# shizukutanaka/Otedama

Measured on AMD Instinct MI355X. Metric: hashes/sec (whole node) SHA-256d + scrypt at 1/2/4/8 MI355X; p50 share latency, higher is better.
Workload: dtype u32

## Files before the change

### csrc/bindings.cpp

```cpp
#include <pybind11/pybind11.h>
#include <pybind11/stl.h>

#include <array>
#include <atomic>
#include <cstring>
#include <stdexcept>
#include <thread>
#include <tuple>

#include "otedama/aead.h"
#include "otedama/job.h"
#include "otedama/runtime.h"
#include "otedama/trace.h"
#include "otedama/sha256.h"
#include "otedama/sv2_frame.h"
#include "otedama/clock_bounds.h"
#include "otedama/launch_plan.h"
#include "otedama/search_launch.h"
#include "otedama/work_queue.h"
#include "otedama/x11.h"

namespace py = pybind11;
using namespace otedama;

// ... 286 lines not shown
                       &status);
        }
        py::list frames(k);
        for (size_t i = 0; i < k; ++i) {
          const Sv2FrameRec& r = recs[i];
          frames[i] = py::make_tuple(r.extension_type, r.msg_type, r.offset, r.length);
        }
        return py::make_tuple(frames, consumed, status);
      },
      py::arg("buf"), py::arg("max_frame"),
      "Split complete SV2 frames: ([(extension_type, msg_type, payload_offset, payload_length)], consumed, status)");
  m.def("cpu_scan_sha256d", [](const py::bytes& h, const py::bytes& t, uint32_t start, uint64_t count) {
    std::string hs = need(h, 80, "header"), ts = need(t, 32, "target");
    std::vector<uint32_t> hits;
    {
      py::gil_scoped_release r;
      hits = cpu_scan_sha256d(reinterpret_cast<const uint8_t*>(hs.data()), reinterpret_cast<const uint8_t*>(ts.data()),
                              start, count);
    }
    return hits;
  }, py::arg("header"), py::arg("target"), py::arg("start"), py::arg("count"));
  m.def("cpu_scan_method", &cpu_scan_method);
  m.def("_cpu_scan_lanes", [](int lanes, const py::bytes& h, const py::bytes& t, uint32_t start, uint64_t count) {
    std::string hs = need(h, 80, "header"), ts = need(t, 32, "target");
    std::vector<uint32_t> hits;
    {
      py::gil_scoped_release r;
      hits = cpu_scan_sha256d_lanes(lanes, reinterpret_cast<const uint8_t*>(hs.data()),
                                    reinterpret_cast<const uint8_t*>(ts.data()), start, count);
    }
    return hits;
  });
  m.def("merkle_root", [](const py::dict& job, uint64_t en2) {
    auto j = make_job(job); uint8_t root[32];
    merkle_root_from_coinbase(*j, en2, root);
    return to_bytes(root, 32);
  });
  m.def("variant_header", [](const py::dict& job, uint64_t v) {
    auto j = make_job(job);
    uint8_t hdr[80]; uint32_t ver, nt; uint64_t en2;
    j->variant_header(v, hdr, &ver, &nt, &en2);
    return py::make_tuple(to_bytes(hdr, 80), ver, nt, en2);
  });
  m.def("variant_space", [](const py::dict& job) { return make_job(job)->variant_space(); });

  m.def("sha256d_prepare", [](const py::bytes& h, const py::bytes& t) {
    std::string hs = need(h, 80, "header"), ts = need(t, 32, "target");
    Sha256dParams p;
    sha256d_prepare(reinterpret_cast<const uint8_t*>(hs.data()), reinterpret_cast<const uint8_t*>(ts.data()), &p);
    return py::bytes(reinterpret_cast<const char*>(&p), sizeof p);
  });
  m.attr("SHA256D_MAX_K") = kSha256dMaxK;
  {
    py::list ks;
    for (int k = 2; k <= kSha256dMaxK; ++k)
      if (sha256d_k_floor(k) == k) ks.append(k);
    m.attr("SHA256D_K_VALUES") = py::tuple(ks);
  }
  m.def("sha256d_prepare_k", [](const py::list& headers, const py::bytes& t) {
    std::string ts = need(t, 32, "target");
    std::vector<std::string> hs;
    for (auto& h : headers) hs.push_back(need(h.cast<py::bytes>(), 80, "header"));
    std::vector<const uint8_t*> ptrs;
    for (auto& h : hs) ptrs.push_back(reinterpret_cast<const uint8_t*>(h.data()));
    Sha256dParamsK p;
    if (!sha256d_prepare_k(ptrs.data(), (int)ptrs.size(), reinterpret_cast<const uint8_t*>(ts.data()), &p))
      throw std::invalid_argument("need K headers (K in SHA256D_K_VALUES) with identical bytes 64..75");
    return py::bytes(reinterpret_cast<const char*>(&p), sizeof p);
  }, py::arg("headers"), py::arg("target"));
  m.attr("SHA256D_V_GROUP") = kSha256dVGroup;
  m.attr("SHA256D_V2_GROUP") = kSha256dV2Group;
  m.def("sha256d_prepare_v", [](const py::list& headers, const py::bytes& t) {
    std::string ts = need(t, 32, "target");
    std::vector<std::string> hs;
    for (auto& h : headers) hs.push_back(need(h.cast<py::bytes>(), 80, "header"));
    std::vector<const uint8_t*> ptrs;
    for (auto& h : hs) ptrs.push_back(reinterpret_cast<const uint8_t*>(h.data()));
    Sha256dParamsV p;
    std::vector<Sha256dVariant> vars(hs.size());
    if (!sha256d_prepare_v(ptrs.data(), (int)ptrs.size(), reinterpret_cast<const uint8_t*>(ts.data()), &p, vars.data()))
      throw std::invalid_argument("need a positive multiple of 64 headers with identical bytes 64..75");
    return py::make_tuple(py::bytes(reinterpret_cast<const char*>(&p), sizeof p),
                          py::bytes(reinterpret_cast<const char*>(vars.data()), vars.size() * sizeof(Sha256dVariant)));
  }, py::arg("headers"), py::arg("target"));
  m.def("scrypt_prepare", [](const py::bytes& h, const py::bytes& t) {
    std::string hs = need(h, 80, "header"), ts = need(t, 32, "target");
    ScryptParams p;
    scrypt_prepare(reinterpret_cast<const uint8_t*>(hs.data()), reinterpret_cast<const uint8_t*>(ts.data()), &p);
    return py::bytes(reinterpret_cast<const char*>(&p), sizeof p);
  });

  m.def("x11_prepare", [](const py::bytes& h, const py::bytes& t) {
    std::string hs = need(h, 80, "header"), ts = need(t, 32, "target");
    X11Params p;
    x11_prepare(reinterpret_cast<const uint8_t*>(hs.data()), reinterpret_cast<const uint8_t*>(ts.data()), &p);
    return py::bytes(reinterpret_cast<const char*>(&p), sizeof p);
  });

  m.def("trace_push", [](const std::string& name) { trace_push(name.c_str()); });
  m.def("trace_pop", [] { trace_pop(); });
  m.def("trace_mark", [](const std::string& name) { trace_mark(name.c_str()); });
  m.def("gpu_device_count", &gpu_device_count);
  m.def("gpu_arch_name", &gpu_arch_name);
  m.def("gpu_cu_count", &gpu_cu_count);
  m.def("scrypt_scratch_bytes", &scrypt_scratch_bytes);
  m.def("maps_range_writable", [](const std::string& maps, uint64_t lo, uint64_t hi) {
    return maps_range_writable(maps, uintptr_t(lo), uintptr_t(hi));
  });
  m.def("launch_sha256d", [](const py::bytes& params, uint32_t base, uint64_t count, uintptr_t out, uint32_t cap,
                             int grid, uintptr_t stream) {
    std::string ps = need(params, sizeof(Sha256dParams), "params");
    Sha256dParams p; std::memcpy(&p, ps.data(), sizeof p);
    if (count == 0 || count > (1ull << 32)) throw std::invalid_argument("count must be in [1, 2^32]");
    if (grid <= 0 || out == 0) throw std::invalid_argument("bad grid / out");
    py_launch_sha256d(p, base, count, out, cap, grid, stream);
  }, py::arg("params"), py::arg("base"), py::arg("count"), py::arg("out"), py::arg("cap"), py::arg("grid"),
     py::arg("stream"));
  m.def("launch_sha256d_k", [](const py::bytes& params, uint32_t base, uint64_t count, uintptr_t out, uint32_t cap,
                               int grid, uintptr_t stream) {
    std::string ps = need(params, sizeof(Sha256dParamsK), "params");
    Sha256dParamsK p; std::memcpy(&p, ps.data(), sizeof p);
    if (p.k < 2 || p.k > kSha256dMaxK) throw std::invalid_argument("bad K");
    if (count == 0 || count > (1ull << 32)) throw std::invalid_argument("count must be in [1, 2^32]");
    if (grid <= 0 || out == 0) throw std::invalid_argument("bad grid / out");
    py_launch_sha256d_k(p, base, count, out, cap, grid, stream);
  }, py::arg("params"), py::arg("base"), py::arg("count"), py::arg("out"), py::arg("cap"), py::arg("grid"),
     py::arg("stream"));
  m.def("launch_sha256d_v", [](const py::bytes& params, uintptr_t vars, uint32_t base, uint64_t count, uintptr_t out,
                               uint32_t cap, int grid, uintptr_t stream, bool occupancy8, int block, int chains) {
    std::string ps = need(params, sizeof(Sha256dParamsV), "params");
    Sha256dParamsV p; std::memcpy(&p, ps.data(), sizeof p);
    p.occupancy8 = occupancy8 ? 1u : 0u;
    if (p.groups == 0 || count == 0 || count > (1ull << 32)) throw std::invalid_argument("bad groups / count");
    if (block != 64 && block != 256) throw std::invalid_argument("block must be 64 or 256 threads");
    if (chains < 1 || chains > 4) throw std::invalid_argument("chains must be 1..4");
    if (p.groups % uint32_t(chains) != 0)
      throw std::invalid_argument("chains variants per lane need a multiple of 64 * chains variants");
    if (grid <= 0 || (uint64_t(grid) * uint32_t(block / 64)) % (p.groups / uint32_t(chains)) != 0 || vars == 0 || out == 0)
      throw std::invalid_argument("the wave count must be a multiple of the variant groups; vars/out must be set");
    py_launch_sha256d_v(p, vars, base, count, out, cap, grid, stream, block, chains);
  }, py::arg("params"), py::arg("vars"), py::arg("base"), py::arg("count"), py::arg("out"), py::arg("cap"),
     py::arg("grid"), py::arg("stream"), py::arg("occupancy8") = false, py::arg("block") = 256, py::arg("chains") = 1);
  m.def("launch_scrypt", [](const py::bytes& params, uint32_t base, uint32_t count, uintptr_t xbuf, uintptr_t scratch,
                            int gap, uintptr_t out, uint32_t cap, int grid, uintptr_t stream) {
    std::string ps = need(params, sizeof(ScryptParams), "params");
    ScryptParams p; std::memcpy(&p, ps.data(), sizeof p);
    if (gap != 1 && gap != 2 && gap != 4 && gap != kScryptCoop && gap != kScryptLaneW8 && gap != kScryptCoop2 &&
        gap != kScryptCoopSplit)
      throw std::invalid_argument("gap must be 1, 2, 4, SCRYPT_COOP or SCRYPT_LANE_W8");
    if (grid <= 0 || out == 0 || xbuf == 0 || scratch == 0 || count == 0) throw std::invalid_argument("bad launch args");
    py_launch_scrypt(p, base, count, xbuf, scratch, gap, out, cap, grid, stream);
  }, py::arg("params"), py::arg("base"), py::arg("count"), py::arg("xbuf"), py::arg("scratch"), py::arg("gap"),
     py::arg("out"), py::arg("cap"), py::arg("grid"), py::arg("stream"));

  m.def("launch_x11_stage", [](const py::bytes& params, int stage, uint32_t base, uintptr_t H, uint32_t stride,
                               uint32_t n, uintptr_t out, uint32_t cap, uintptr_t stream) {
    std::string ps = need(params, sizeof(X11Params), "params");
    X11Params p; std::memcpy(&p, ps.data(), sizeof p);
    if (stage < 0 || stage >= kX11StageCount) throw std::invalid_argument("stage must be in [0, 11)");
    if (H == 0 || n == 0 || stride < n) throw std::invalid_argument("need H != 0, n > 0, stride >= n");
    py_launch_x11_stage(p, stage, base, H, stride, n, out, cap, stream);
  }, py::arg("params"), py::arg("stage"), py::arg("base"), py::arg("H"), py::arg("stride"), py::arg("n"),
     py::arg("out") = 0, py::arg("cap") = 0, py::arg("stream") = 0);
  m.def("launch_x11", [](const py::bytes& params, uint32_t base, uintptr_t H, uint32_t stride, uint32_t n,
                         uintptr_t out, uint32_t cap, uintptr_t stream) {
    std::string ps = need(params, sizeof(X11Params), "params");
    X11Params p; std::memcpy(&p, ps.data(), sizeof p);
    if (H == 0 || n == 0 || stride < n) throw std::invalid_argument("need H != 0, n > 0, stride >= n");
    py_launch_x11(p, base, H, stride, n, out, cap, stream);
  }, py::arg("params"), py::arg("base"), py::arg("H"), py::arg("stride"), py::arg("n"), py::arg("out") = 0,
     py::arg("cap") = 0, py::arg("stream") = 0);

  py::class_<MinerBase, std::shared_ptr<MinerBase>>(m, "Miner")
      .def("start", &MinerBase::start, py::call_guard<py::gil_scoped_release>())
      .def("stop", &MinerBase::stop, py::call_guard<py::gil_scoped_release>())
      .def("set_job", [](MinerBase& self, py::object job) {
        if (job.is_none()) { py::gil_scoped_release r; self.set_job(nullptr); return; }
        auto j = make_job(job.cast<py::dict>());
        py::gil_scoped_release r;
        self.set_job(j);
      })
      .def("poll", [](MinerBase& self, size_t max) {
        std::vector<ShareRecord> v;
        { py::gil_scoped_release r; v = self.poll(max); }
        return shares_to_list(std::move(v));
      }, py::arg("max") = 256)
      .def("stats", [](MinerBase& self) { return stats_to_dict(self.stats()); })
      .def("share_fd", &MinerBase::share_fd,
           "eventfd that becomes readable when shares are queued (read 8 bytes to reset, then poll())")
      .def_property_readonly("device_id", &MinerBase::device_id);

  py::class_<GpuMiner, MinerBase, std::shared_ptr<GpuMiner>>(m, "GpuMiner")
      .def(py::init<int, std::string, uint64_t, int, size_t, int>(), py::arg("device"), py::arg("device_id"),
           py::arg("batch_nonces") = (1ull << 32), py::arg("grid") = 2048, py::arg("queue_cap") = 1024,
           py::arg("sha_variants") = 128);
  py::class_<CpuMiner, MinerBase, std::shared_ptr<CpuMiner>>(m, "CpuMiner")
      .def(py::init<int, std::string, size_t>(), py::arg("threads"), py::arg("device_id") = "cpu-0",
           py::arg("queue_cap") = 1024);

  m.attr("SHA256D_PARAMS_SIZE") = sizeof(Sha256dParams);
  m.attr("SHA256D_V_PARAMS_SIZE") = sizeof(Sha256dParamsV);
  m.attr("SCRYPT_PARAMS_SIZE") = sizeof(ScryptParams);
}
```

### csrc/include/otedama/search_launch.h

```cpp
#pragma once
#include <cstdint>
#include <string>

#include "otedama/hitsink.h"
#include "otedama/job.h"

namespace otedama {

uint64_t scrypt_scratch_bytes(int grid, int gap);

int gpu_device_count();
std::string gpu_arch_name(int device);
int gpu_cu_count(int device);

void py_launch_sha256d(const Sha256dParams& p, uint32_t base, uint64_t count, uintptr_t out, uint32_t cap, int grid,
                       uintptr_t stream);
void py_launch_sha256d_k(const Sha256dParamsK& p, uint32_t base, uint64_t count, uintptr_t out, uint32_t cap, int grid,
                         uintptr_t stream);
void py_launch_sha256d_v(const Sha256dParamsV& p, uintptr_t vars, uint32_t base, uint64_t count, uintptr_t out,
                         uint32_t cap, int grid, uintptr_t stream, int block, int chains);
void py_launch_scrypt(const ScryptParams& p, uint32_t base, uint32_t count, uintptr_t xbuf, uintptr_t scratch, int gap,
                      uintptr_t out, uint32_t cap, int grid, uintptr_t stream);
void py_launch_x11_stage(const X11Params& p, int stage, uint32_t base, uintptr_t H, uint32_t stride, uint32_t n,
                         uintptr_t out, uint32_t cap, uintptr_t stream);
void py_launch_x11(const X11Params& p, uint32_t base, uintptr_t H, uint32_t stride, uint32_t n, uintptr_t out,
                   uint32_t cap, uintptr_t stream);

}

#ifdef __HIPCC__
#include <hip/hip_runtime.h>

namespace otedama {

hipError_t launch_sha256d_search(const Sha256dParams& p, uint32_t base, uint64_t count, const HitSink& sink, int grid,
                                 hipStream_t stream);
hipError_t launch_sha256d_search_k(const Sha256dParamsK& p, uint32_t base, uint64_t count, const HitSink& sink,
                                   int grid, hipStream_t stream);
hipError_t launch_sha256d_search_v(const Sha256dParamsV& p, const Sha256dVariant* vars, uint32_t base, uint64_t count,
                                   const HitSink& sink, int grid, hipStream_t stream, int block = 256, int chains = 1);

hipError_t launch_scrypt_search(const ScryptParams& p, uint32_t base, uint32_t count, void* xbuf, void* scratch,
                                int gap, const HitSink& sink, int grid, hipStream_t stream);

}
#endif
```

### csrc/kernels/scrypt_search.hip

```cpp
#include <hip/hip_runtime.h>

#include <cstdint>

#include "cdna_bitops.h"
#include "hitsink_dev.h"
#include <cstdlib>
#include <cstring>

#include "otedama/job.h"
#include "otedama/search_launch.h"

namespace {

using namespace otedama_dev;

__device__ __forceinline__ uint32_t bswap(uint32_t x) { return __builtin_bswap32(x); }

__device__ __forceinline__ void salsa20_8(uint32_t B[16]) {
  uint32_t x0 = B[0], x1 = B[1], x2 = B[2], x3 = B[3], x4 = B[4], x5 = B[5], x6 = B[6], x7 = B[7];
  uint32_t x8 = B[8], x9 = B[9], x10 = B[10], x11 = B[11], x12 = B[12], x13 = B[13], x14 = B[14], x15 = B[15];
#pragma unroll
  for (int i = 0; i < 8; i += 2) {
    x4 ^= rol(x0 + x12, 7);   x8 ^= rol(x4 + x0, 9);    x12 ^= rol(x8 + x4, 13);   x0 ^= rol(x12 + x8, 18);
    x9 ^= rol(x5 + x1, 7);    x13 ^= rol(x9 + x5, 9);   x1 ^= rol(x13 + x9, 13);   x5 ^= rol(x1 + x13, 18);
    x14 ^= rol(x10 + x6, 7);  x2 ^= rol(x14 + x10, 9);  x6 ^= rol(x2 + x14, 13);   x10 ^= rol(x6 + x2, 18);
    x3 ^= rol(x15 + x11, 7);  x7 ^= rol(x3 + x15, 9);   x11 ^= rol(x7 + x3, 13);   x15 ^= rol(x11 + x7, 18);
    x1 ^= rol(x0 + x3, 7);    x2 ^= rol(x1 + x0, 9);    x3 ^= rol(x2 + x1, 13);    x0 ^= rol(x3 + x2, 18);
    x6 ^= rol(x5 + x4, 7);    x7 ^= rol(x6 + x5, 9);    x4 ^= rol(x7 + x6, 13);    x5 ^= rol(x4 + x7, 18);
    x11 ^= rol(x10 + x9, 7);  x8 ^= rol(x11 + x10, 9);  x9 ^= rol(x8 + x11, 13);   x10 ^= rol(x9 + x8, 18);
    x12 ^= rol(x15 + x14, 7); x13 ^= rol(x12 + x15, 9); x14 ^= rol(x13 + x12, 13); x15 ^= rol(x14 + x13, 18);
  }
  B[0] += x0; B[1] += x1; B[2] += x2; B[3] += x3; B[4] += x4; B[5] += x5; B[6] += x6; B[7] += x7;
  B[8] += x8; B[9] += x9; B[10] += x10; B[11] += x11; B[12] += x12; B[13] += x13; B[14] += x14; B[15] += x15;
}

__device__ __forceinline__ void blockmix(uint32_t X[32]) {
#pragma unroll
  for (int k = 0; k < 16; ++k) X[k] ^= X[16 + k];
  salsa20_8(X);
#pragma unroll
  for (int k = 0; k < 16; ++k) X[16 + k] ^= X[k];
  salsa20_8(X + 16);
}

__device__ __forceinline__ void store_entry(uint4* __restrict__ dst, const uint32_t X[32]) {
#pragma unroll
  for (int q = 0; q < 8; ++q) dst[q] = make_uint4(X[4 * q], X[4 * q + 1], X[4 * q + 2], X[4 * q + 3]);
}
__device__ __forceinline__ void load_entry(const uint4* __restrict__ src, uint32_t T[32]) {
#pragma unroll
  for (int q = 0; q < 8; ++q) {
    const uint4 v = src[q];
    T[4 * q] = v.x; T[4 * q + 1] = v.y; T[4 * q + 2] = v.z; T[4 * q + 3] = v.w;
  }
}

__device__ __forceinline__ void hmac_states(const uint32_t key[8], uint32_t istate[8], uint32_t ostate[8]) {
  uint32_t blk[16];
#pragma unroll
  for (int i = 0; i < 8; ++i) blk[i] = key[i] ^ 0x36363636u;
#pragma unroll
  for (int i = 8; i < 16; ++i) blk[i] = 0x36363636u;
#pragma unroll
  for (int i = 0; i < 8; ++i) istate[i] = kSha256IVd[i];
  sha256_compress(istate, blk);
#pragma unroll
  for (int i = 0; i < 8; ++i) blk[i] = key[i] ^ 0x5c5c5c5cu;
#pragma unroll
  for (int i = 8; i < 16; ++i) blk[i] = 0x5c5c5c5cu;
#pragma unroll
  for (int i = 0; i < 8; ++i) ostate[i] = kSha256IVd[i];
  sha256_compress(ostate, blk);
}

__device__ __forceinline__ void hmac_outer(const uint32_t ostate[8], const uint32_t digest[8], uint32_t out[8]) {
  uint32_t blk[16];
#pragma unroll
  for (int i = 0; i < 8; ++i) blk[i] = digest[i];
  blk[8] = 0x80000000u;
#pragma unroll
  for (int i = 9; i < 15; ++i) blk[i] = 0u;
  blk[15] = 768u;
#pragma unroll
  for (int i = 0; i < 8; ++i) out[i] = ostate[i];
  sha256_compress(out, blk);
}

__device__ __forceinline__ void scrypt_pbkdf_in(const otedama::ScryptParams& p, uint32_t nonce, uint32_t X[32]) {
  uint32_t hdrbe[20];
#pragma unroll
  for (int i = 0; i < 19; ++i) hdrbe[i] = bswap(p.hdr[i]);
  hdrbe[19] = bswap(nonce);
  uint32_t key[8];
#pragma unroll
  for (int i = 0; i < 8; ++i) key[i] = p.hmid[i];
  {
    uint32_t blk[16] = {hdrbe[16], hdrbe[17], hdrbe[18], hdrbe[19], 0x80000000u, 0, 0, 0, 0, 0, 0, 0, 0, 0, 0, 640u};
    sha256_compress(key, blk);
  }
  uint32_t istate[8], ostate[8];
  hmac_states(key, istate, ostate);
  uint32_t ist2[8];
#pragma unroll
  for (int i = 0; i < 8; ++i) ist2[i] = istate[i];
  sha256_compress(ist2, hdrbe);
#pragma unroll
  for (int blkno = 1; blkno <= 4; ++blkno) {
    uint32_t st[8];
#pragma unroll
    for (int i = 0; i < 8; ++i) st[i] = ist2[i];
    uint32_t blk[16] = {hdrbe[16], hdrbe[17], hdrbe[18], hdrbe[19], uint32_t(blkno), 0x80000000u,
                        0, 0, 0, 0, 0, 0, 0, 0, 0, (64u + 84u) * 8u};
    sha256_compress(st, blk);
    uint32_t t[8];
    hmac_outer(ostate, st, t);
#pragma unroll
    for (int i = 0; i < 8; ++i) X[8 * (blkno - 1) + i] = bswap(t[i]);
  }
}

__device__ __forceinline__ uint32_t scrypt_pbkdf_out(const otedama::ScryptParams& p, uint32_t nonce,
                                                     const uint32_t X[32]) {
  uint32_t key[8];
#pragma unroll
  for (int i = 0; i < 8; ++i) key[i] = p.hmid[i];
  {
    uint32_t blk[16] = {bswap(p.hdr[16]), bswap(p.hdr[17]), bswap(p.hdr[18]), bswap(nonce), 0x80000000u,
                        0, 0, 0, 0, 0, 0, 0, 0, 0, 0, 640u};
    sha256_compress(key, blk);
  }
  uint32_t istate[8], ostate[8];
  hmac_states(key, istate, ostate);
  uint32_t st[8];
#pragma unroll
  for (int i = 0; i < 8; ++i) st[i] = istate[i];
  uint32_t blk[16];
#pragma unroll
  for (int i = 0; i < 16; ++i) blk[i] = bswap(X[i]);
  sha256_compress(st, blk);
#pragma unroll
  for (int i = 0; i < 16; ++i) blk[i] = bswap(X[16 + i]);
  sha256_compress(st, blk);
  uint32_t tail[16] = {1u, 0x80000000u, 0, 0, 0, 0, 0, 0, 0, 0, 0, 0, 0, 0, 0, (64u + 132u) * 8u};
  sha256_compress(st, tail);
  uint32_t out[8];
  hmac_outer(ostate, st, out);
  return out[7];
}

template <int GAP>
__device__ __forceinline__ void scrypt_romix(uint32_t X[32], uint4* __restrict__ Vw, uint32_t lane) {
  for (int i = 0; i < 1024; ++i) {
    if (i % GAP == 0) store_entry(Vw + ((uint64_t(i / GAP) * 64u + lane) << 3), X);
    blockmix(X);
  }
  for (int i = 0; i < 1024; ++i) {
    const uint32_t j = X[16] & 1023u;
    uint32_t T[32];
    load_entry(Vw + ((uint64_t(j / GAP) * 64u + lane) << 3), T);
    if constexpr (GAP > 1) {
// ... 237 lines not shown
        __builtin_amdgcn_make_buffer_rsrc(V + hw * (1024ull * 64u * 8u), (short)0, 1024 * 64 * 128, 0x00020000);
    uint32_t X[32];
    load_entry(xbuf + (h << 3), X);
    const uint32_t w1 = it1 < 1024u ? it1 : 1024u;
    for (uint32_t i = it0; i < w1; ++i) {
      coop_store_entry(X, rh, tile, lane, i);
      blockmix(X);
    }
    for (uint32_t i = it0 > 1024u ? it0 : 1024u; i < it1; ++i) {
      coop_v4u R[4];
      coop_issue<LCPOL>(X, rh, tile, lane, R);
      coop_consume(X, tile, lane, R);
      blockmix(X);
    }
    store_entry(xbuf + (h << 3), X);
  }
}

template <int LCPOL>
__global__ __launch_bounds__(256) __attribute__((amdgpu_waves_per_eu(4, 4))) void otd_scrypt_romix_coop2(
    uint32_t count, uint4* __restrict__ xbuf, uint4* __restrict__ V) {
  __shared__ uint4 tiles[4 * 256];
  const uint32_t lane = threadIdx.x & 63u;
  const uint64_t wave0 = (uint64_t(blockIdx.x) * blockDim.x + threadIdx.x) >> 6;
  const uint64_t nwaves = (uint64_t(gridDim.x) * blockDim.x) >> 6;
  const uint64_t wslot = (uint64_t(__builtin_amdgcn_readfirstlane(uint32_t(wave0 >> 32))) << 32) |
                         uint64_t(__builtin_amdgcn_readfirstlane(uint32_t(wave0)));
  uint4* VA = V + wslot * (2ull * 1024 * 64 * 8);
  uint4* VB = VA + 1024ull * 64 * 8;
  const __amdgpu_buffer_rsrc_t rsA = __builtin_amdgcn_make_buffer_rsrc(VA, (short)0, 1024 * 64 * 128, 0x00020000);
  const __amdgpu_buffer_rsrc_t rsB = __builtin_amdgcn_make_buffer_rsrc(VB, (short)0, 1024 * 64 * 128, 0x00020000);
  uint4* tile = tiles + __builtin_amdgcn_readfirstlane(threadIdx.x >> 6) * 256;
  for (uint64_t w = wslot; w * 128 < count; w += nwaves) {
    const uint64_t ia = w * 128 + lane, ib = ia + 64;
    uint32_t XA[32], XB[32];
    load_entry(xbuf + (ia << 3), XA);
    load_entry(xbuf + (ib << 3), XB);
    scrypt_romix_coop2<LCPOL>(XA, XB, rsA, rsB, tile, lane);
    store_entry(xbuf + (ia << 3), XA);
    store_entry(xbuf + (ib << 3), XB);
  }
}

__global__ __launch_bounds__(256) __attribute__((amdgpu_waves_per_eu(8, 8))) void otd_scrypt_romix_w8(
    uint32_t count, uint4* __restrict__ xbuf, uint4* __restrict__ V) {
  const uint64_t slot = uint64_t(blockIdx.x) * blockDim.x + threadIdx.x;
  const uint64_t nslots = uint64_t(gridDim.x) * blockDim.x;
  uint4* Vw = V + (slot >> 6) * (1024ull * 64u * 8u);
  const uint32_t lane = uint32_t(slot & 63u);
  for (uint64_t i = slot; i < count; i += nslots) {
    uint32_t X[32];
    load_entry(xbuf + (i << 3), X);
    scrypt_romix<1>(X, Vw, lane);
    store_entry(xbuf + (i << 3), X);
  }
}

extern "C" __global__ __launch_bounds__(256) void otd_scrypt_pbkdf_out(const otedama::ScryptParams p, uint32_t base,
                                                                       uint32_t count, const uint4* __restrict__ xbuf,
                                                                       const otedama::HitSink sink) {
  const uint32_t i = blockIdx.x * blockDim.x + threadIdx.x;
  if (i >= count) return;
  if (abort_newer(abort_peek(sink), sink.epoch)) return;
  uint32_t X[32];
  load_entry(xbuf + (uint64_t(i) << 3), X);
  const uint32_t h7 = scrypt_pbkdf_out(p, base + i, X);
  if (bswap(h7) <= p.target_hi) hit_publish(sink, base + i, 0u);
}

template __global__ void otd_scrypt_romix<1>(uint32_t, uint4*, uint4*);
template __global__ void otd_scrypt_romix<2>(uint32_t, uint4*, uint4*);
template __global__ void otd_scrypt_romix<4>(uint32_t, uint4*, uint4*);

namespace otedama {

uint64_t scrypt_scratch_bytes(int grid, int gap) {
  if (gap == kScryptCoop2) return uint64_t(grid) * 512ull * 1024ull * 128ull;
  if (gap == kScryptCoop || gap == kScryptLaneW8 || gap == kScryptCoopSplit) gap = 1;
  return uint64_t(grid) * 256ull * (1024ull / uint64_t(gap)) * 128ull;
}

static bool scrypt_write_polls() {
  static const bool on = [] {
    const char* v = std::getenv("OTEDAMA_SCRYPT_POLL");
    return !(v && v[0] == '0');
  }();
  return on;
}

static uint32_t scrypt_segments() {
  const char* v = std::getenv("OTEDAMA_SCRYPT_SEGMENTS");
  if (!v || !v[0]) return 0;
  const long x = std::strtol(v, nullptr, 10);
  return uint32_t(x < 1 ? 1 : (x > 64 ? 64 : x));
}

static int scrypt_seg_grid(int grid) {
  const char* v = std::getenv("OTEDAMA_SCRYPT_SEG_GRID");
  if (!v || !v[0]) return grid;
  int cap = 0;
  if (std::strcmp(v, "resident") == 0) {
    int dev = 0, cus = 0;
    if (hipGetDevice(&dev) != hipSuccess ||
        hipDeviceGetAttribute(&cus, hipDeviceAttributeMultiprocessorCount, dev) != hipSuccess || cus <= 0)
      return grid;
    cap = cus * 8;
  } else {
    cap = int(std::strtol(v, nullptr, 10));
  }
  return cap > 0 && cap < grid ? cap : grid;
}

hipError_t launch_scrypt_search(const ScryptParams& p, uint32_t base, uint32_t count, void* xbuf, void* scratch,
                                int gap, const HitSink& sink, int grid, hipStream_t stream) {
  uint4* X = static_cast<uint4*>(xbuf);
  uint4* V = static_cast<uint4*>(scratch);
  const int eg = int((count + 255) / 256);
  const uint32_t count64 = (count + 63u) & ~63u;
  if (gap == kScryptCoopSplit && uint64_t(count64) > uint64_t(grid) * 256u) return hipErrorInvalidValue;
  hipLaunchKernelGGL(otd_scrypt_pbkdf_in, dim3(eg), dim3(256), 0, stream, p, base, count, X);
  switch (gap) {
    case kScryptCoop:
      if (scrypt_segments() > 0 && uint64_t(count64) <= uint64_t(grid) * 256u) {
        const uint32_t S = scrypt_segments();
        const int sg = scrypt_seg_grid(grid);
        for (uint32_t k = 0; k < S; ++k)
          hipLaunchKernelGGL(otd_scrypt_romix_coop_seg<2>, dim3(sg), dim3(256), 0, stream, count64, X, V,
                             2048u * k / S, 2048u * (k + 1) / S, sink);
      } else if (scrypt_write_polls())
        hipLaunchKernelGGL((otd_scrypt_romix_coop<2, 64>), dim3(grid), dim3(256), 0, stream, count64, X, V, sink);
      else
        hipLaunchKernelGGL((otd_scrypt_romix_coop<2, 1024>), dim3(grid), dim3(256), 0, stream, count64, X, V, sink);
      break;
    case kScryptLaneW8:
      hipLaunchKernelGGL(otd_scrypt_romix_w8, dim3(grid), dim3(256), 0, stream, count, X, V);
      break;
    case kScryptCoopSplit:
      hipLaunchKernelGGL((otd_scrypt_romix_coop_phase<2, 1>), dim3(grid), dim3(256), 0, stream, count64, X, V);
      hipLaunchKernelGGL((otd_scrypt_romix_coop_phase<2, 2>), dim3(grid), dim3(256), 0, stream, count64, X, V);
      break;
    case kScryptCoop2:
      hipLaunchKernelGGL(otd_scrypt_romix_coop2<2>, dim3(grid), dim3(256), 0, stream, (count + 127u) & ~127u, X, V);
      break;
    case 1: hipLaunchKernelGGL(otd_scrypt_romix<1>, dim3(grid), dim3(256), 0, stream, count, X, V); break;
    case 2: hipLaunchKernelGGL(otd_scrypt_romix<2>, dim3(grid), dim3(256), 0, stream, count, X, V); break;
    case 4: hipLaunchKernelGGL(otd_scrypt_romix<4>, dim3(grid), dim3(256), 0, stream, count, X, V); break;
    default: return hipErrorInvalidValue;
  }
  hipLaunchKernelGGL(otd_scrypt_pbkdf_out, dim3(eg), dim3(256), 0, stream, p, base, count, X, sink);
  return hipGetLastError();
}

}
```

### otedama_amd/ops/search.py

```python
from __future__ import annotations

from dataclasses import dataclass

import torch

from otedama_amd.ops.native import require_native

from otedama_amd.ops.tuning import (
    SCRYPT_BLOCKS_PER_CU,
    SHA256D_BLOCKS_PER_CU,
    SHA256D_K_BLOCKS_PER_CU,
    SHA256D_V2_BLOCKS_PER_CU,
    SHA256D_V_BLOCKS_PER_CU,
)


def _device_index(device) -> int:
    d = torch.device(device)
    return 0 if d.index is None else d.index


def default_grid(device, blocks_per_cu: int) -> int:
    n = require_native()
    cus = n.gpu_cu_count(_device_index(device)) or 256
    return cus * blocks_per_cu


@dataclass
class SearchResult:
    buf: torch.Tensor
    cap: int

    def count(self) -> int:
        return int(self.buf[0].item()) & 0xFFFFFFFF

    def nonces(self) -> list[int]:
        host = self.buf.cpu().tolist()
        n = min(host[0] & 0xFFFFFFFF, self.cap)
        return [x & 0xFFFFFFFF for x in host[1 : 1 + n]]


class Sha256dSearch:

    def __init__(self, device="cuda:0", cap: int = 1024, grid: int | None = None):
        self.native = require_native()
        self.device = torch.device(device)
        self.cap = cap
        self.grid = grid or default_grid(self.device, SHA256D_BLOCKS_PER_CU)
        self.out = torch.zeros(1 + cap, dtype=torch.int32, device=self.device)

    def prepare(self, header80: bytes, target32: bytes) -> bytes:
        return self.native.sha256d_prepare(header80, target32)

    def launch(self, params: bytes, base: int = 0, count: int = 1 << 32, out: torch.Tensor | None = None,
               stream: torch.cuda.Stream | None = None) -> SearchResult:
        out = self.out if out is None else out
        if out.numel() < 1 + self.cap or out.dtype != torch.int32 or out.device != self.device:
            raise ValueError("out must be an int32 tensor of >= 1+cap elements on the search device")
        stream = stream or torch.cuda.current_stream(self.device)
        with torch.cuda.stream(stream):
            out[:1].zero_()
        self.native.launch_sha256d(params, base & 0xFFFFFFFF, int(count), out.data_ptr(), self.cap, self.grid,
                                   stream.cuda_stream)
        return SearchResult(out, self.cap)

    def search(self, header80: bytes, target32: bytes, base: int = 0, count: int = 1 << 32) -> list[int]:
        r = self.launch(self.prepare(header80, target32), base, count)
        torch.cuda.synchronize(self.device)
        return r.nonces()


@dataclass
class SearchResultK:
    buf: torch.Tensor
    cap: int

    def count(self) -> int:
        return int(self.buf[0].item()) & 0xFFFFFFFF

    def hits(self) -> list[tuple[int, int]]:
        host = self.buf.cpu().tolist()
        n = min(host[0] & 0xFFFFFFFF, self.cap)
        return [(host[1 + 2 * i] & 0xFFFFFFFF, host[2 + 2 * i]) for i in range(n)]


class Sha256dSearchK:

    def __init__(self, device="cuda:0", k: int = 4, cap: int = 1024, grid: int | None = None):
        self.native = require_native()
        if k not in self.native.SHA256D_K_VALUES:
            raise ValueError(f"k must be one of {self.native.SHA256D_K_VALUES}")
        self.k = k
        self.device = torch.device(device)
        self.cap = cap
        self.grid = grid or default_grid(self.device, SHA256D_K_BLOCKS_PER_CU)
        self.out = torch.zeros(1 + 2 * cap, dtype=torch.int32, device=self.device)

    def prepare(self, headers: list[bytes], target32: bytes) -> bytes:
        if len(headers) != self.k:
            raise ValueError(f"need exactly {self.k} headers")
        return self.native.sha256d_prepare_k(list(headers), target32)

    def launch(self, params: bytes, base: int = 0, count: int = 1 << 32, out: torch.Tensor | None = None,
               stream: torch.cuda.Stream | None = None) -> SearchResultK:
        out = self.out if out is None else out
        if out.numel() < 1 + 2 * self.cap or out.dtype != torch.int32 or out.device != self.device:
            raise ValueError("out must be an int32 tensor of >= 1+2*cap elements on the search device")
        stream = stream or torch.cuda.current_stream(self.device)
        with torch.cuda.stream(stream):
            out[:1].zero_()
        self.native.launch_sha256d_k(params, base & 0xFFFFFFFF, int(count), out.data_ptr(), self.cap, self.grid,
                                     stream.cuda_stream)
        return SearchResultK(out, self.cap)

    def search(self, headers: list[bytes], target32: bytes, base: int = 0, count: int = 1 << 32) -> list[tuple[int, int]]:
        r = self.launch(self.prepare(headers, target32), base, count)
        torch.cuda.synchronize(self.device)
        return r.hits()


@dataclass
class PreparedV:
    params: bytes
    vars: torch.Tensor
    n: int


class Sha256dSearchV:

    def __init__(self, device="cuda:0", cap: int = 1024, grid: int | None = None, occupancy8: bool = True,
                 block: int = 256, chains: int = 1):
        self.native = require_native()
        if chains not in (1, 2, 3, 4):
            raise ValueError("chains must be 1..4")
        self.chains = chains
        self.group = self.native.SHA256D_V_GROUP * chains
        self.occupancy8 = occupancy8
        if block not in (64, 256):
            raise ValueError("block must be 64 or 256 threads")
        self.block = block
        self.device = torch.device(device)
        self.cap = cap
        self.grid = grid or default_grid(self.device, SHA256D_V_BLOCKS_PER_CU)
        self.out = torch.zeros(1 + 2 * cap, dtype=torch.int32, device=self.device)

    def prepare(self, headers: list[bytes], target32: bytes) -> PreparedV:
        if not headers or len(headers) % self.group:
            raise ValueError(f"need a positive multiple of {self.group} headers")
        groups = len(headers) // self.group
        waves = self.grid * self.block // 64
        if waves % groups:
            raise ValueError(f"the wave count ({waves}) must be a multiple of the variant groups ({groups})")
        params, table = self.native.sha256d_prepare_v(list(headers), target32)
        vars_dev = torch.frombuffer(bytearray(table), dtype=torch.uint8).to(self.device)
        return PreparedV(params, vars_dev, len(headers))

    def launch(self, prep: PreparedV, base: int = 0, count: int = 1 << 32, out: torch.Tensor | None = None,
               stream: torch.cuda.Stream | None = None) -> SearchResultK:
        out = self.out if out is None else out
        if out.numel() < 1 + 2 * self.cap or out.dtype != torch.int32 or out.device != self.device:
            raise ValueError("out must be an int32 tensor of >= 1+2*cap elements on the search device")
        if prep.vars.device != self.device:
            raise ValueError("variant table must live on the search device")
        if prep.vars.numel() != prep.n * 72 or len(prep.params) != self.native.SHA256D_V_PARAMS_SIZE:
            raise ValueError("prepared table does not match its parameter block")
        cur = torch.cuda.current_stream(self.device)
        if stream is None:
            stream = cur
        elif stream != cur:
            stream.wait_stream(cur)
        with torch.cuda.stream(stream):
            out[:1].zero_()
        self.launch_into(prep, base, count, out, stream)
        return SearchResultK(out, self.cap)

    def launch_into(self, prep: PreparedV, base: int, count: int, out: torch.Tensor, stream) -> None:
        self.native.launch_sha256d_v(prep.params, prep.vars.data_ptr(), base & 0xFFFFFFFF, int(count),
                                     out.data_ptr(), self.cap, self.grid, stream.cuda_stream, self.occupancy8,
                                     self.block, self.chains)

    def search(self, headers: list[bytes], target32: bytes, base: int = 0, count: int = 1 << 32) -> list[tuple[int, int]]:
        r = self.launch(self.prepare(headers, target32), base, count)
        torch.cuda.synchronize(self.device)
        return r.hits()


class ScryptSearch:

    def __init__(self, device="cuda:0", cap: int = 1024, grid: int | None = None, gap: int = 1,
                 lanes_per_slot: int = 1, kernel: str = "coop"):
        self.native = require_native()
        codes = {"coop": self.native.SCRYPT_COOP, "coop2": self.native.SCRYPT_COOP2,
                 "split": self.native.SCRYPT_COOP_SPLIT}
        if kernel not in ("coop", "coop2", "split", "lane"):
            raise ValueError(f"kernel must be 'coop', 'coop2', 'split' or 'lane', got {kernel!r}")
        if kernel in codes and gap == 1:
            gap = codes[kernel]
        self.kernel = {v: k for k, v in codes.items()}.get(gap, "lane")
        if self.kernel == "split" and lanes_per_slot != 1:
            raise ValueError("the split kernel holds one hash per lane slot")
        self.device = torch.device(device)
        self.cap = cap
        self.gap = gap
        self.grid = grid or default_grid(self.device, SCRYPT_BLOCKS_PER_CU // (2 if self.kernel == "coop2" else 1))
        self.batch = self.grid * 256 * lanes_per_slot * (2 if self.kernel == "coop2" else 1)
        nbytes = self.native.scrypt_scratch_bytes(self.grid, gap)
        self.scratch = torch.empty(nbytes, dtype=torch.uint8, device=self.device)
        self.xbuf = torch.empty(self.batch * 128, dtype=torch.uint8, device=self.device)
        self.out = torch.zeros(1 + cap, dtype=torch.int32, device=self.device)

    @property
    def scratch_bytes(self) -> int:
        return self.scratch.numel()

    def prepare(self, header80: bytes, target32: bytes) -> bytes:
        return self.native.scrypt_prepare(header80, target32)

    def launch(self, params: bytes, base: int = 0, count: int | None = None,
               stream: torch.cuda.Stream | None = None) -> SearchResult:
        count = self.batch if count is None else count
        if not 0 < count <= self.batch:
            raise ValueError(f"count must be in [1, {self.batch}]")
        stream = stream or torch.cuda.current_stream(self.device)
        with torch.cuda.stream(stream):
            self.out[:1].zero_()
        self.native.launch_scrypt(params, base & 0xFFFFFFFF, int(count), self.xbuf.data_ptr(),
                                  self.scratch.data_ptr(), self.gap, self.out.data_ptr(), self.cap, self.grid,
                                  stream.cuda_stream)
        return SearchResult(self.out, self.cap)

    def search(self, header80: bytes, target32: bytes, base: int = 0, count: int | None = None) -> list[int]:
        r = self.launch(self.prepare(header80, target32), base, count)
        torch.cuda.synchronize(self.device)
        return r.nonces()


X11_BATCH = 1 << 23


class X11Search:

    def __init__(self, device="cuda:0", cap: int = 1024, batch: int = X11_BATCH):
        self.native = require_native()
        self.device = torch.device(device)
        self.cap = cap
        self.batch = int(batch)
        if not 0 < self.batch <= 1 << 26:
            raise ValueError("batch must be in [1, 2^26]")
        self.H = torch.empty(8 * self.batch, dtype=torch.int64, device=self.device)
        self.out = torch.zeros(1 + cap, dtype=torch.int32, device=self.device)

    def prepare(self, header80: bytes, target32: bytes) -> bytes:
        return self.native.x11_prepare(header80, target32)

    def launch(self, params: bytes, base: int = 0, count: int | None = None,
               stream: torch.cuda.Stream | None = None) -> SearchResult:
        count = self.batch if count is None else count
        if not 0 < count <= self.batch:
            raise ValueError(f"count must be in [1, {self.batch}]")
        stream = stream or torch.cuda.current_stream(self.device)
        with torch.cuda.stream(stream):
            self.out[:1].zero_()
        self.native.launch_x11(params, base & 0xFFFFFFFF, self.H.data_ptr(), self.batch, int(count),
                               self.out.data_ptr(), self.cap, stream.cuda_stream)
        return SearchResult(self.out, self.cap)

    def search(self, header80: bytes, target32: bytes, base: int = 0, count: int | None = None) -> list[int]:
        r = self.launch(self.prepare(header80, target32), base, count)
        torch.cuda.synchronize(self.device)
        return r.nonces()

    def trace(self, header80: bytes, base: int, count: int) -> list[torch.Tensor]:
        if not 0 < count <= self.batch:
            raise ValueError(f"count must be in [1, {self.batch}]")
        params = self.prepare(header80, bytes(32))
        stream = torch.cuda.current_stream(self.device)
        planes = self.H.view(8, self.batch)
        out = []
        for st in range(self.native.X11_STAGES):
            self.native.launch_x11_stage(params, st, base & 0xFFFFFFFF, self.H.data_ptr(), self.batch, int(count),
                                         0, 0, stream.cuda_stream)
            torch.cuda.synchronize(self.device)
            words = planes[:, :count].t().contiguous().cpu()
            out.append(words.view(torch.uint8).reshape(count, 64))
        return out
```

Measured before the change: 19.45 billion.

## Pipeline scrypt search across two streams with staggered half-grid phases

Adds a ScryptPipeline that splits the coop scrypt batch into two halves, each run on its own non-blocking stream as pbkdf_in, two romix segments and pbkdf_out. The second half's ROMix is held back until the first half finishes its first segment, so the memory-heavy write and read phases of the two halves overlap. Per-half hit buffers are double-buffered by call parity and merged into the caller's output by a small kernel. It also skips the caller-stream wait when params and stream are unchanged, so successive launches can overlap. This costs extra events, stream synchronisation, a merge kernel per launch and more complex ordering.

```diff
diff --git a/csrc/bindings.cpp b/csrc/bindings.cpp
--- a/csrc/bindings.cpp
+++ b/csrc/bindings.cpp
@@ -462,6 +462,18 @@
     py_launch_scrypt(p, base, count, xbuf, scratch, gap, out, cap, grid, stream);
   }, py::arg("params"), py::arg("base"), py::arg("count"), py::arg("xbuf"), py::arg("scratch"), py::arg("gap"),
      py::arg("out"), py::arg("cap"), py::arg("grid"), py::arg("stream"));
+  py::class_<ScryptPipeline>(m, "ScryptPipeline")
+      .def(py::init<int, uintptr_t, uintptr_t, int, uint32_t>(), py::arg("device"), py::arg("xbuf"),
+           py::arg("scratch"), py::arg("grid"), py::arg("cap"))
+      .def("launch", [](ScryptPipeline& self, const py::bytes& params, uint32_t base, uint32_t count, uintptr_t out,
+                        uintptr_t stream) {
+        std::string ps = need(params, sizeof(ScryptParams), "params");
+        ScryptParams p; std::memcpy(&p, ps.data(), sizeof p);
+        self.launch(p, base, count, out, stream);
+      }, py::arg("params"), py::arg("base"), py::arg("count"), py::arg("out"), py::arg("stream"))
+      .def("synchronize", [](ScryptPipeline& self) { py::gil_scoped_release r; self.synchronize(); })
+      .def_property_readonly("last_launch_flags", &ScryptPipeline::last_launch_flags)
+      .def_property_readonly("launches", &ScryptPipeline::launches);
 
   m.def("launch_x11_stage", [](const py::bytes& params, int stage, uint32_t base, uintptr_t H, uint32_t stride,
                                uint32_t n, uintptr_t out, uint32_t cap, uintptr_t stream) {
diff --git a/csrc/include/otedama/search_launch.h b/csrc/include/otedama/search_launch.h
--- a/csrc/include/otedama/search_launch.h
+++ b/csrc/include/otedama/search_launch.h
@@ -26,6 +26,22 @@
 void py_launch_x11(const X11Params& p, uint32_t base, uintptr_t H, uint32_t stride, uint32_t n, uintptr_t out,
                    uint32_t cap, uintptr_t stream);
 
+class ScryptPipeline {
+ public:
+  ScryptPipeline(int device, uintptr_t xbuf, uintptr_t scratch, int grid, uint32_t cap);
+  ~ScryptPipeline();
+  ScryptPipeline(const ScryptPipeline&) = delete;
+  ScryptPipeline& operator=(const ScryptPipeline&) = delete;
+  void launch(const ScryptParams& p, uint32_t base, uint32_t count, uintptr_t out, uintptr_t caller_stream);
+  void synchronize();
+  uint32_t last_launch_flags() const;
+  uint64_t launches() const;
+
+ private:
+  struct Impl;
+  Impl* d_;
+};
+
 }
 
 #ifdef __HIPCC__
diff --git a/csrc/kernels/scrypt_search.hip b/csrc/kernels/scrypt_search.hip
--- a/csrc/kernels/scrypt_search.hip
+++ b/csrc/kernels/scrypt_search.hip
@@ -6,6 +6,8 @@
 #include "hitsink_dev.h"
 #include <cstdlib>
 #include <cstring>
+#include <stdexcept>
+#include <string>
 
 #include "otedama/job.h"
 #include "otedama/search_launch.h"
@@ -549,3 +551,164 @@
 }
 
 }
+
+extern "C" __global__ __launch_bounds__(256) void otd_scrypt_merge_hits(uint32_t* __restrict__ a,
+                                                                        uint32_t* __restrict__ b,
+                                                                        uint32_t* __restrict__ out, uint32_t cap) {
+  __shared__ uint32_t first;
+  const uint32_t na = a[0], nb = b ? b[0] : 0u;
+  if (threadIdx.x == 0) first = atomicAdd(out, na + nb);
+  __syncthreads();
+  const uint32_t ka = na < cap ? na : cap, kb = nb < cap ? nb : cap;
+  for (uint32_t i = threadIdx.x; i < ka + kb; i += blockDim.x) {
+    const uint64_t dst = uint64_t(first) + i;
+    if (dst < cap) out[1 + dst] = i < ka ? a[1 + i] : b[1 + (i - ka)];
+  }
+  if (threadIdx.x == 0) {
+    a[0] = 0u;
+    if (b) b[0] = 0u;
+  }
+}
+
+namespace otedama {
+
+namespace {
+void pipe_check(hipError_t e, const char* what) {
+  if (e != hipSuccess) throw std::runtime_error(std::string("HIP error ") + hipGetErrorString(e) + " at " + what);
+}
+#define OTD_PIPE(call) pipe_check((call), #call)
+
+struct DeviceScope {
+  int prev = -1, dev;
+  explicit DeviceScope(int d) : dev(d) {
+    OTD_PIPE(hipGetDevice(&prev));
+    if (prev != dev) OTD_PIPE(hipSetDevice(dev));
+  }
+  ~DeviceScope() {
+    if (prev != dev && prev >= 0) (void)hipSetDevice(prev);
+  }
+};
+}
+
+struct ScryptPipeline::Impl {
+  int device = 0, half_grid = 0;
+  uint32_t half_lanes = 0, cap = 0;
+  uint4* xbuf[2] = {nullptr, nullptr};
+  uint4* pad[2] = {nullptr, nullptr};
+  hipStream_t stream[2] = {nullptr, nullptr};
+  uint32_t* slots = nullptr;
+  hipEvent_t caller_ev = nullptr, phase_ev = nullptr;
+  hipEvent_t done_ev[2][2] = {{nullptr, nullptr}, {nullptr, nullptr}};
+  hipEvent_t merged_ev[2] = {nullptr, nullptr};
+  bool merged_set[2] = {false, false};
+  ScryptParams prev{};
+  hipStream_t prev_caller = nullptr;
+  bool started = false;
+  bool staggered = false;
+  uint64_t calls = 0;
+  uint32_t flags = 0;
+
+  uint32_t* slot(int half, int parity) const { return slots + (size_t(half) * 2 + size_t(parity)) * (1 + size_t(cap)); }
+
+  void release() {
+    for (auto& s : stream)
+      if (s) (void)hipStreamSynchronize(s);
+    for (auto& s : stream)
+      if (s) (void)hipStreamDestroy(s), s = nullptr;
+    for (hipEvent_t* e : {&caller_ev, &phase_ev, &done_ev[0][0], &done_ev[0][1], &done_ev[1][0], &done_ev[1][1],
+                          &merged_ev[0], &merged_ev[1]})
+      if (*e) (void)hipEventDestroy(*e), *e = nullptr;
+    if (slots) (void)hipFree(slots), slots = nullptr;
+  }
+};
+
+ScryptPipeline::ScryptPipeline(int device, uintptr_t xbuf, uintptr_t scratch, int grid, uint32_t cap) : d_(new Impl) {
+  try {
+    if (grid < 2 || (grid & 1) || xbuf == 0 || scratch == 0 || cap == 0)
+      throw std::invalid_argument("ScryptPipeline: an even grid >= 2, xbuf, scratch and cap > 0 are required");
+    Impl& d = *d_;
+    d.device = device;
+    d.half_grid = grid / 2;
+    d.half_lanes = uint32_t(d.half_grid) * 256u;
+    d.cap = cap;
+    for (int h = 0; h < 2; ++h) {
+      d.xbuf[h] = reinterpret_cast<uint4*>(xbuf + uint64_t(h) * d.half_lanes * 128ull);
+      d.pad[h] = reinterpret_cast<uint4*>(scratch + uint64_t(h) * scrypt_scratch_bytes(d.half_grid, kScryptCoop));
+    }
+    DeviceScope scope(device);
+    for (auto& s : d.stream) OTD_PIPE(hipStreamCreateWithFlags(&s, hipStreamNonBlocking));
+    for (hipEvent_t* e : {&d.caller_ev, &d.phase_ev, &d.done_ev[0][0], &d.done_ev[0][1], &d.done_ev[1][0],
+                          &d.done_ev[1][1], &d.merged_ev[0], &d.merged_ev[1]})
+      OTD_PIPE(hipEventCreateWithFlags(e, hipEventDisableTiming));
+    const size_t bytes = 4 * (1 + size_t(cap)) * sizeof(uint32_t);
+    OTD_PIPE(hipMalloc(reinterpret_cast<void**>(&d.slots), bytes));
+    OTD_PIPE(hipMemset(d.slots, 0, bytes));
+  } catch (...) {
+    d_->release();
+    delete d_;
+    throw;
+  }
+}
+
+ScryptPipeline::~ScryptPipeline() {
+  d_->release();
+  delete d_;
+}
+
+void ScryptPipeline::synchronize() {
+  for (auto& s : d_->stream) OTD_PIPE(hipStreamSynchronize(s));
+}
+
+uint32_t ScryptPipeline::last_launch_flags() const { return d_->flags; }
+uint64_t ScryptPipeline::launches() const { return d_->calls; }
+
+void ScryptPipeline::launch(const ScryptParams& p, uint32_t base, uint32_t count, uintptr_t out_ptr,
+                            uintptr_t caller_stream) {
+  Impl& d = *d_;
+  if (count == 0 || uint64_t(count) > 2ull * d.half_lanes || out_ptr == 0)
+    throw std::invalid_argument("ScryptPipeline::launch: count must be in [1, grid * 256] and out set");
+  DeviceScope scope(d.device);
+  hipStream_t caller = reinterpret_cast<hipStream_t>(caller_stream);
+  uint32_t* out = reinterpret_cast<uint32_t*>(out_ptr);
+  const int parity = int(d.calls & 1u);
+  const uint32_t n[2] = {count < d.half_lanes ? count : d.half_lanes, count > d.half_lanes ? count - d.half_lanes : 0u};
+  const bool wait_caller = !d.started || caller != d.prev_caller || std::memcmp(&p, &d.prev, sizeof p) != 0;
+  const bool wait_phase = n[1] > 0 && (wait_caller || !d.staggered);
+  if (wait_caller) OTD_PIPE(hipEventRecord(d.caller_ev, caller));
+  for (int h = 0; h < 2; ++h) {
+    if (n[h] == 0) continue;
+    hipStream_t s = d.stream[h];
+    const uint32_t n64 = (n[h] + 63u) & ~63u;
+    const int eg = int((n[h] + 255u) / 256u);
+    const uint32_t hbase = base + (h ? n[0] : 0u);
+    HitSink sink;
+    sink.out = d.slot(h, parity);
+    sink.cap = d.cap;
+    sink.words = 1;
+    if (wait_caller) OTD_PIPE(hipStreamWaitEvent(s, d.caller_ev, 0));
+    if (d.merged_set[parity]) OTD_PIPE(hipStreamWaitEvent(s, d.merged_ev[parity], 0));
+    hipLaunchKernelGGL(otd_scrypt_pbkdf_in, dim3(eg), dim3(256), 0, s, p, hbase, n[h], d.xbuf[h]);
+    if (h == 1 && wait_phase) OTD_PIPE(hipStreamWaitEvent(s, d.phase_ev, 0));
+    hipLaunchKernelGGL(otd_scrypt_romix_coop_seg<2>, dim3(d.half_grid), dim3(256), 0, s, n64, d.xbuf[h], d.pad[h], 0u,
+                       1024u, sink);
+    if (h == 0 && wait_phase) OTD_PIPE(hipEventRecord(d.phase_ev, s));
+    hipLaunchKernelGGL(otd_scrypt_romix_coop_seg<2>, dim3(d.half_grid), dim3(256), 0, s, n64, d.xbuf[h], d.pad[h],
+                       1024u, 2048u, sink);
+    hipLaunchKernelGGL(otd_scrypt_pbkdf_out, dim3(eg), dim3(256), 0, s, p, hbase, n[h], d.xbuf[h], sink);
+    OTD_PIPE(hipEventRecord(d.done_ev[h][parity], s));
+    OTD_PIPE(hipStreamWaitEvent(caller, d.done_ev[h][parity], 0));
+  }
+  hipLaunchKernelGGL(otd_scrypt_merge_hits, dim3(1), dim3(256), 0, caller, d.slot(0, parity),
+                     n[1] ? d.slot(1, parity) : static_cast<uint32_t*>(nullptr), out, d.cap);
+  OTD_PIPE(hipEventRecord(d.merged_ev[parity], caller));
+  d.merged_set[parity] = true;
+  d.prev = p;
+  d.prev_caller = caller;
+  d.started = true;
+  d.staggered = n[1] > 0;
+  d.flags = (wait_caller ? 1u : 0u) | (wait_phase ? 2u : 0u) | (n[1] ? 4u : 0u);
+  ++d.calls;
+  OTD_PIPE(hipGetLastError());
+}
+
+}
diff --git a/otedama_amd/ops/search.py b/otedama_amd/ops/search.py
--- a/otedama_amd/ops/search.py
+++ b/otedama_amd/ops/search.py
@@ -1,5 +1,6 @@
 from __future__ import annotations
 
+import os
 from dataclasses import dataclass
 
 import torch
@@ -208,6 +209,29 @@
         self.scratch = torch.empty(nbytes, dtype=torch.uint8, device=self.device)
         self.xbuf = torch.empty(self.batch * 128, dtype=torch.uint8, device=self.device)
         self.out = torch.zeros(1 + cap, dtype=torch.int32, device=self.device)
+        self._pipe = None
+        if (self.kernel == "coop" and lanes_per_slot == 1 and self.grid >= 2 and self.grid % 2 == 0
+                and os.environ.get("OTEDAMA_SCRYPT_HALVES", "1")[:1] != "0"
+                and not os.environ.get("OTEDAMA_SCRYPT_SEGMENTS")):
+            torch.cuda.synchronize(self.device)
+            self._pipe = self.native.ScryptPipeline(_device_index(self.device), self.xbuf.data_ptr(),
+                                                    self.scratch.data_ptr(), self.grid, cap)
+
+    @property
+    def pipelined(self) -> bool:
+        return self._pipe is not None
+
+    def close(self) -> None:
+        pipe, self._pipe = self._pipe, None
+        if pipe is not None:
+            pipe.synchronize()
+            del pipe
+
+    def __del__(self):
+        try:
+            self.close()
+        except Exception:
+            pass
 
     @property
     def scratch_bytes(self) -> int:
@@ -224,6 +248,9 @@
         stream = stream or torch.cuda.current_stream(self.device)
         with torch.cuda.stream(stream):
             self.out[:1].zero_()
+        if self._pipe is not None:
+            self._pipe.launch(params, base & 0xFFFFFFFF, int(count), self.out.data_ptr(), stream.cuda_stream)
+            return SearchResult(self.out, self.cap)
         self.native.launch_scrypt(params, base & 0xFFFFFFFF, int(count), self.xbuf.data_ptr(),
                                   self.scratch.data_ptr(), self.gap, self.out.data_ptr(), self.cap, self.grid,
                                   stream.cuda_stream)
```

After: 19.45 billion (median of 2 runs). No clear change (+0.0%).
